# happyjin/Gaussian_process

Measured on AMD Instinct MI355X. Metric: GP-fit+predict sec and achieved fp64 TFLOP/s, N=65536 d=8, 1/2/4/8 MI355X, higher is better.
Workload: dtype f64

## Files before the change

gaussian_process_amd/csrc/gemm_dma.hip:

```cpp
#include <algorithm>
#include <cstdlib>
#include <type_traits>

#include "gpmi_internal.h"
#include "gpmi_plan.h"
#include <atomic>
#include <mutex>

namespace gpmi {

typedef double d4 __attribute__((ext_vector_type(4)));
typedef double d2 __attribute__((ext_vector_type(2)));

#define GPMI_LDS __attribute__((address_space(3)))
#define GPMI_GLB __attribute__((address_space(1)))
#define GPMI_CONST __attribute__((address_space(4)))

struct GemmDmaDev {
    double* C;
    const double* A;
    const double* B;
    int64_t ldc, lda, ldb;
    int Tm, Tn;
    int nchunks;
    int lower;
    int64_t diag_off;
    const int32_t* row_ncols;
    int row_block_tiles;
    const int64_t* b_block_off;
    int b_block_tiles;
    int S, logS, SM, SN, tri, nsuper;
    int pair;
    int sprefix[DMA_MAX_SM + 1];
    unsigned long long* stamps;
    int dbg;
    struct PersistSlot* slot;
    int nblocks;
};

struct PersistSlot {
    unsigned ctr[8];
    unsigned done;
    unsigned pad[7];
};

template <class PT>
__device__ __forceinline__ bool dma_block_to_tile(const PT& p, int b, int& ti, int& tj) {
    return plan_block_to_tile(p, b, ti, tj);
}

__device__ __forceinline__ bool dma_map_tile(const GemmDmaDev& p, int& ti, int& tj) {
    return dma_block_to_tile(p, blockIdx.x, ti, tj);
}

constexpr int DMA_TM = PLAN_TILE, DMA_TN = PLAN_TILE;
template <class PT>
__device__ __forceinline__ bool dma_tile_live(const PT& p, int ti, int tj) {
    return plan_tile_live(p, ti, tj, p.row_ncols);
}
constexpr int DMA_STAGE_SLOTS = (DMA_TM + DMA_TN) * 8;
constexpr int DMA_STAGES = 3;

constexpr unsigned TICKET_NONE = 0xFFFFFFFFu;

template <class PT>
__device__ __forceinline__ unsigned ticket_draw(const PT& p, int xcd) {
    const unsigned per = (unsigned)p.nblocks >> 3;
#pragma unroll 1
    for (int t = 0; t < 8; ++t) {
        const int x = (xcd + t) & 7;
        if (t && __hip_atomic_load(&p.slot->ctr[x], __ATOMIC_RELAXED, __HIP_MEMORY_SCOPE_AGENT) >= per) continue;
        const unsigned w = atomicAdd(&p.slot->ctr[x], 1u);
        if (w < per) return w * 8u + (unsigned)x;
    }
    return TICKET_NONE;
}

template <int MI, bool DBG, bool TICKET = false>
__device__ __forceinline__ void gemm_nt_dma_body(const GemmDmaDev& p) {
    constexpr int NWAVES = 16 / MI;
    constexpr int DPW = 32 / NWAVES;
    constexpr int RPW = DMA_TM / NWAVES;
    constexpr int NFR = MI + 4;
    const int dbg = DBG ? p.dbg : 0;
    extern __shared__ __attribute__((aligned(16))) char smem_raw[];
    const int tid = threadIdx.x;
    volatile GPMI_LDS int* mbox = (volatile GPMI_LDS int*)(smem_raw + DMA_STAGES * DMA_STAGE_SLOTS * 16);
    unsigned blk = blockIdx.x, nxt_blk = TICKET_NONE;
    int par = 0;
    if constexpr (TICKET) {
        if (tid == 0) mbox[0] = (int)ticket_draw(p, (int)(blockIdx.x & 7));
        __syncthreads();
        blk = (unsigned)__builtin_amdgcn_readfirstlane(mbox[0]);
        par = 1;
    }
  for (;;) {
    int ti = 0, tj = 0;
    bool live;
    if constexpr (TICKET) {
        if (blk == TICKET_NONE) break;
        live = dma_block_to_tile(p, (int)blk, ti, tj) && dma_tile_live(p, ti, tj);
        live = __builtin_amdgcn_readfirstlane(live ? 1 : 0) != 0;
        ti = __builtin_amdgcn_readfirstlane(ti);
        tj = __builtin_amdgcn_readfirstlane(tj);
    } else {
        live = dma_map_tile(p, ti, tj) && dma_tile_live(p, ti, tj);
        if (!live) return;
    }
   if (live) {
    unsigned long long st0 = 0, st1 = 0, st2 = 0, st3 = 0;
    if (DBG && (dbg & 16)) st0 = clock64();
    const int lane = tid & 63;
    const int wave = __builtin_amdgcn_readfirstlane(tid >> 6);
    const int wr = (wave >> 1) * (16 * MI);
    const int wc = (wave & 1) * 64;
    const int fr = lane & 15;
    const int fg = lane >> 4;

    const int drow = lane >> 3;
    const int dkp = (lane & 7) ^ (drow & 7);
    const double* a_src = p.A + ((int64_t)ti * DMA_TM + RPW * wave + drow) * p.lda + dkp * 2;
    int64_t b_row0 = (int64_t)tj * DMA_TN * p.ldb;
    if (p.b_block_off) {
        const int blk = tj / p.b_block_tiles;
        b_row0 = p.b_block_off[blk] + (int64_t)(tj - blk * p.b_block_tiles) * DMA_TN * p.ldb;
    }
    const double* b_src = p.B + b_row0 + (int64_t)(RPW * wave + drow) * p.ldb + dkp * 2;
    const int64_t a_step = 8 * p.lda, b_step = 8 * p.ldb;
    GPMI_LDS char* lds = (GPMI_LDS char*)smem_raw;
    const int a_dst = (RPW * wave) * 128;
    const int b_dst = DMA_TM * 128 + (RPW * wave) * 128;

    auto issue_dma_one = [&](int chunk, int q) {
        const int st = chunk % DMA_STAGES;
        GPMI_LDS char* base = lds + st * (DMA_STAGE_SLOTS * 16);
        const int k0 = chunk * 16;
        if (q < DPW / 2)
            __builtin_amdgcn_global_load_lds((const GPMI_GLB void*)(a_src + q * a_step + k0),
                                             (GPMI_LDS void*)(base + a_dst + q * 1024), 16, 0, 0);
        else
            __builtin_amdgcn_global_load_lds((const GPMI_GLB void*)(b_src + (q - DPW / 2) * b_step + k0),
                                             (GPMI_LDS void*)(base + b_dst + (q - DPW / 2) * 1024), 16, 0, 0);
    };
    auto issue_dma = [&](int chunk) {
#pragma unroll
        for (int q = 0; q < DPW; ++q) issue_dma_one(chunk, q);
    };

    const int x7 = fr & 7;
    const int sl0 = fr * 8 + (fg ^ x7);
    const int sl1 = fr * 8 + ((4 + fg) ^ x7);
    const d2* smem = reinterpret_cast<const d2*>(smem_raw);
    auto read_one = [&](int chunk, int half, int q, d2 (&fa)[MI], d2 (&fb)[4]) {
        const d2* sa = smem + (chunk % DMA_STAGES) * DMA_STAGE_SLOTS;
        const d2* sb = sa + DMA_TM * 8;
        const int sl = half ? sl1 : sl0;
        if (q < MI) fa[q] = sa[(wr + 16 * q) * 8 + sl];
        else fb[q - MI] = sb[(wc + 16 * (q - MI)) * 8 + sl];
    };
    auto read_frags = [&](int chunk, int half, d2 (&fa)[MI], d2 (&fb)[4]) {
#pragma unroll
        for (int q = 0; q < NFR; ++q) read_one(chunk, half, q, fa, fb);
    };

    d4 acc[MI][4];
#pragma unroll
    for (int i = 0; i < MI; ++i)
#pragma unroll
        for (int j = 0; j < 4; ++j) acc[i][j] = d4{0., 0., 0., 0.};
    const int nch = p.nchunks;
    d2 fa0[MI], fb0[4], fa1[MI], fb1[4];
    issue_dma(0);
    if (nch > 1) {
        issue_dma(1);
        if constexpr (DPW == 8) asm volatile("s_waitcnt vmcnt(8)" ::: "memory");
        else asm volatile("s_waitcnt vmcnt(4)" ::: "memory");
    } else {
        asm volatile("s_waitcnt vmcnt(0)" ::: "memory");
    }
    __builtin_amdgcn_s_barrier();
    read_frags(0, 0, fa0, fb0);
    if (DBG && (dbg & 16)) st1 = clock64();

#define GPMI_MFMA_X(FA, FB, T) acc[(T) >> 2][(T) & 3] = __builtin_amdgcn_mfma_f64_16x16x4f64(FA[(T) >> 2].x, FB[(T) & 3].x, acc[(T) >> 2][(T) & 3], 0, 0, 0)
#define GPMI_MFMA_Y(FA, FB, T) acc[(T) >> 2][(T) & 3] = __builtin_amdgcn_mfma_f64_16x16x4f64(FA[(T) >> 2].y, FB[(T) & 3].y, acc[(T) >> 2][(T) & 3], 0, 0, 0)
#define GPMI_FENCE() __builtin_amdgcn_sched_barrier(0)
    constexpr int NT = 4 * MI;
    constexpr int NSLOT = NT / 2;

// ... 62 lines not shown
    }
    constexpr int NB3 = MI < 3 ? MI : 3;
    double cv[NB3][4][4];
#pragma unroll
    for (int i = 0; i < NB3; ++i)
#pragma unroll
        for (int j = 0; j < 4; ++j)
#pragma unroll
            for (int v = 0; v < 4; ++v) cv[i][j][v] = *c_ptr(i, j, v);
    if (DBG && (dbg & 16)) {
        asm volatile("s_waitcnt vmcnt(0)" ::: "memory");
        st3 = clock64();
    }
#pragma unroll
    for (int i = 0; i < MI; ++i) {
#pragma unroll
        for (int j = 0; j < 4; ++j)
#pragma unroll
            for (int v = 0; v < 4; ++v) *c_ptr(i, j, v) = cv[i % NB3][j][v] - acc[i][j][v];
        if (i == 0 && MI > 3) {
#pragma unroll
            for (int j = 0; j < 4; ++j)
#pragma unroll
                for (int v = 0; v < 4; ++v) cv[0][j][v] = *c_ptr(3, j, v);
        }
    }
    if (DBG && (dbg & 16)) {
        asm volatile("s_waitcnt vmcnt(0)" ::: "memory");
        const unsigned long long st4 = clock64();
        if (lane == 0 && blockIdx.x < 4096) {
            unsigned long long* o = p.stamps + ((size_t)blockIdx.x * 4 + (wave & 3)) * 4;
            o[0] = st1 - st0; o[1] = st2 - st1; o[2] = st3 - st2; o[3] = st4 - st3;
        }
    }
   }
    if constexpr (!TICKET) {
        return;
    } else {
        if (tid == 0) {
            if (!live) nxt_blk = ticket_draw(p, (int)(blockIdx.x & 7));
            mbox[par] = (int)nxt_blk;
        }
        __syncthreads();
        blk = (unsigned)__builtin_amdgcn_readfirstlane(mbox[par]);
        par ^= 1;
    }
  }
    if constexpr (TICKET) {
        if (tid == 0) {
            __threadfence();
            const unsigned old = atomicAdd(&p.slot->done, 1u);
            if (old == gridDim.x - 1) {
#pragma unroll
                for (int x = 0; x < 8; ++x) p.slot->ctr[x] = 0;
                p.slot->done = 0;
                __threadfence();
            }
        }
    }
}

template <int MI, bool DBG>
__global__ __launch_bounds__(1024 / MI, (MI == 4) ? 2 : 3) void gemm_nt_dma_kernel(const GemmDmaDev p) {
    gemm_nt_dma_body<MI, DBG>(p);
}

__global__ __launch_bounds__(512, 3) void chol_trailing_update_dma_kernel(const GemmDmaDev p) {
    gemm_nt_dma_body<2, false>(p);
}

constexpr int TALL_TM = 2 * DMA_TM;
constexpr int TALL_STAGE_SLOTS = (TALL_TM + DMA_TN) * 8;
constexpr int TALL_STAGES = 2;
constexpr size_t TALL_LDS = (size_t)TALL_STAGES * TALL_STAGE_SLOTS * 16;
static_assert(TALL_LDS == (size_t)DMA_STAGES * DMA_STAGE_SLOTS * 16, "the tall form keeps the LDS footprint");

template <bool DBG>
__device__ __forceinline__ void gemm_nt_dma_tall_body(const GemmDmaDev& p) {
    constexpr int DPW = 6;
    const int dbg = DBG ? p.dbg : 0;
    extern __shared__ __attribute__((aligned(16))) char smem_raw[];
    const int tid = threadIdx.x;
    int ti = 0, tj = 0;
    if (!dma_block_to_tile(p, blockIdx.x, ti, tj)) return;
    bool l0, l1;
    plan_pair_live(p, ti, tj, p.row_ncols, l0, l1);
    ti = __builtin_amdgcn_readfirstlane(ti);
    tj = __builtin_amdgcn_readfirstlane(tj);
    const bool live0 = __builtin_amdgcn_readfirstlane(l0 ? 1 : 0) != 0;
    const bool live1 = __builtin_amdgcn_readfirstlane(l1 ? 1 : 0) != 0;
    if (!live0 && !live1) return;
    unsigned long long st0 = 0, st1 = 0, st2 = 0, st3 = 0;
    if (DBG && (dbg & 16)) st0 = clock64();
    const int lane = tid & 63;
    const int wave = __builtin_amdgcn_readfirstlane(tid >> 6);
    const bool mine = (wave >> 2) ? live1 : live0;
    const int wr = (wave >> 1) * 64;
    const int wc = (wave & 1) * 64;
    const int fr = lane & 15;
    const int fg = lane >> 4;

    const int drow = lane >> 3;
    const int dkp = (lane & 7) ^ (drow & 7);
    const int arow = 32 * wave - ((ti + 1 >= p.Tm && wave >= 4) ? DMA_TM : 0);
    const double* a_row = p.A + ((int64_t)ti * DMA_TM + arow) * p.lda;
    int64_t b_row0 = (int64_t)tj * DMA_TN * p.ldb;
    if (p.b_block_off) {
        const int blk = tj / p.b_block_tiles;
        b_row0 = p.b_block_off[blk] + (int64_t)(tj - blk * p.b_block_tiles) * DMA_TN * p.ldb;
    }
    const double* b_row = p.B + b_row0 + (int64_t)(16 * wave) * p.ldb;
    const unsigned a_lane = (unsigned)((drow * p.lda + dkp * 2) * 8);
    const unsigned b_lane = (unsigned)((drow * p.ldb + dkp * 2) * 8);
    const int64_t a_step = 8 * p.lda, b_step = 8 * p.ldb;
    GPMI_LDS char* lds = (GPMI_LDS char*)smem_raw;
    const int a_dst = (32 * wave) * 128;
    const int b_dst = TALL_TM * 128 + (16 * wave) * 128;
    auto issue_dma_one = [&](int chunk, int q) {
        GPMI_LDS char* base = lds + (chunk & 1) * (TALL_STAGE_SLOTS * 16);
        const int k0 = chunk * 16;
        unsigned off = q < 4 ? a_lane : b_lane;
        asm volatile("" : "+v"(off));
        if (q < 4)
            __builtin_amdgcn_global_load_lds((const GPMI_GLB void*)((const char*)(a_row + q * a_step + k0) + off),
                                             (GPMI_LDS void*)(base + a_dst + q * 1024), 16, 0, 0);
        else
            __builtin_amdgcn_global_load_lds((const GPMI_GLB void*)((const char*)(b_row + (q - 4) * b_step + k0) + off),
                                             (GPMI_LDS void*)(base + b_dst + (q - 4) * 1024), 16, 0, 0);
    };

    const int x7 = fr & 7;
    const int sl0 = fr * 8 + (fg ^ x7);
    const int sl1 = fr * 8 + ((4 + fg) ^ x7);
    const d2* smem = reinterpret_cast<const d2*>(smem_raw);
    auto read_a = [&](int chunk, int half, int i) -> d2 {
        return smem[(chunk & 1) * TALL_STAGE_SLOTS + (wr + 16 * i) * 8 + (half ? sl1 : sl0)];
    };
    auto read_b = [&](int chunk, int half, int j) -> d2 {
        return smem[(chunk & 1) * TALL_STAGE_SLOTS + TALL_TM * 8 + (wc + 16 * j) * 8 + (half ? sl1 : sl0)];
    };

    d4 acc[4][4];
#pragma unroll
    for (int i = 0; i < 4; ++i)
#pragma unroll
        for (int j = 0; j < 4; ++j) acc[i][j] = d4{0., 0., 0., 0.};
    const int nch = p.nchunks;

#define GPMI_MFMA_X(FA, FB, T) acc[(T) >> 2][(T) & 3] = __builtin_amdgcn_mfma_f64_16x16x4f64(FA[(T) >> 2].x, FB[(T) & 3].x, acc[(T) >> 2][(T) & 3], 0, 0, 0)
#define GPMI_MFMA_Y(FA, FB, T) acc[(T) >> 2][(T) & 3] = __builtin_amdgcn_mfma_f64_16x16x4f64(FA[(T) >> 2].y, FB[(T) & 3].y, acc[(T) >> 2][(T) & 3], 0, 0, 0)
#define GPMI_FENCE() __builtin_amdgcn_sched_barrier(0)
    auto kloop = [&](auto live_tag) {
        constexpr bool LIVE = decltype(live_tag)::value;
        d2 fa[4], fb0[4], fb1[4];
#pragma unroll
        for (int q = 0; q < DPW; ++q) issue_dma_one(0, q);
        if (nch > 1) {
#pragma unroll
            for (int q = 0; q < DPW; ++q) issue_dma_one(1, q);
            asm volatile("s_waitcnt vmcnt(6)" ::: "memory");
        } else {
            asm volatile("s_waitcnt vmcnt(0)" ::: "memory");
        }
        __builtin_amdgcn_s_barrier();
        if constexpr (LIVE) {
#pragma unroll
            for (int i = 0; i < 4; ++i) fa[i] = read_a(0, 0, i);
// ... 478 lines not shown
#pragma unroll
        for (int j = 0; j < 2; ++j)
#pragma unroll
            for (int v = 0; v < 4; ++v) *c_ptr(i, j, v) = cv[i][j][v] - acc[i][j][v];
}

bool gemm_small_eligible(const GemmArgs& a) {
    return a.mode == 0 && a.M % SM_T == 0 && a.N % SM_T == 0 && a.K % 16 == 0 && a.K >= 16 && !a.row_ncols && !a.b_block_off;
}

hipError_t launch_gemm_nt_small(hipStream_t s, const GemmArgs& a) {
    GemmSmallDev p;
    p.C = a.C; p.A = a.A; p.B = a.B; p.ldc = a.ldc; p.lda = a.lda; p.ldb = a.ldb;
    p.Tm = (int)(a.M / SM_T); p.Tn = (int)(a.N / SM_T); p.nchunks = (int)(a.K / 16);
    p.lower = a.lower; p.diag_off = a.diag_off;
    constexpr size_t lds8 = (size_t)8 * SM_STAGE_SLOTS * 16, lds3 = (size_t)3 * SM_STAGE_SLOTS * 16;
    static PerDeviceOnce once;
    const hipError_t ea = once.run([&]() -> hipError_t {
        return hipFuncSetAttribute((const void*)gemm_nt_small_kernel<8>, hipFuncAttributeMaxDynamicSharedMemorySize, (int)lds8);
    });
    if (ea != hipSuccess) return ea;
    if (t_small_shallow) hipLaunchKernelGGL(gemm_nt_small_kernel<3>, dim3((unsigned)(p.Tm * p.Tn)), dim3(256), lds3, s, p);
    else hipLaunchKernelGGL(gemm_nt_small_kernel<8>, dim3((unsigned)(p.Tm * p.Tn)), dim3(256), lds8, s, p);
    return hipGetLastError();
}

struct PersistPool {
    static constexpr int SLOTS = 16384;
    PersistSlot* base = nullptr;
    int groups = 0;
    std::atomic<unsigned> head{0};
    PersistSlot* next() { return base + (head.fetch_add(1, std::memory_order_relaxed) % SLOTS); }
};

static PersistPool* persist_pool() {
    static std::mutex mu;
    static PersistPool pools[16];
    int dev = 0;
    if (hipGetDevice(&dev) != hipSuccess || dev < 0 || dev >= 16) return nullptr;
    PersistPool& pl = pools[dev];
    std::lock_guard<std::mutex> lock(mu);
    if (!pl.base) {
        hipDeviceProp_t prop;
        if (hipGetDeviceProperties(&prop, dev) != hipSuccess) return nullptr;
        void* q = nullptr;
        if (hipMalloc(&q, sizeof(PersistSlot) * PersistPool::SLOTS) != hipSuccess) return nullptr;
        if (hipMemset(q, 0, sizeof(PersistSlot) * PersistPool::SLOTS) != hipSuccess) { (void)hipFree(q); return nullptr; }
        pl.groups = (prop.multiProcessorCount / 8) * 8;
        if (pl.groups < 8) { (void)hipFree(q); return nullptr; }
        const void* fns[] = {(const void*)gemm_nt_dma_persist_kernel, (const void*)chol_trailing_update_persist_kernel,
                             (const void*)gemm_nt_dma_ticket_kernel, (const void*)chol_trailing_update_ticket_kernel};
        for (const void* f : fns)
            if (hipFuncSetAttribute(f, hipFuncAttributeMaxDynamicSharedMemorySize,
                                    (int)(DMA_STAGES * DMA_STAGE_SLOTS * 16 + 16)) != hipSuccess) { (void)hipFree(q); return nullptr; }
        pl.base = static_cast<PersistSlot*>(q);
    }
    return &pl;
}

bool gemm_dma_eligible(const GemmArgs& a) {
    return a.mode == 0 && a.N % 128 == 0 && a.M % 128 == 0 && a.K % 16 == 0 && a.K >= 32;
}

hipError_t launch_gemm_nt_dma(hipStream_t s, const GemmArgs& a) {
    GemmDmaDev p;
    p.C = a.C; p.A = a.A; p.B = a.B;
    p.ldc = a.ldc; p.lda = a.lda; p.ldb = a.ldb;
    p.Tm = (int)(a.M / 128); p.Tn = (int)(a.N / 128);
    p.nchunks = (int)(a.K / 16);
    p.lower = a.lower; p.diag_off = a.diag_off;
    p.row_ncols = a.row_ncols; p.row_block_tiles = a.row_block_tiles > 0 ? a.row_block_tiles : 1;
    p.b_block_off = a.b_block_off;
    p.b_block_tiles = a.b_block_off ? (int)(a.b_block_rows / 128) : 1;
    if (a.b_block_off && (a.b_block_rows <= 0 || a.b_block_rows % 128)) return hipErrorInvalidValue;
    const Tuning& tn = tuning();
    TilePlan plan;
    if (!plan_tiles(plan, p.Tm, p.Tn, a.lower, a.diag_off, a.row_ncols != nullptr, a.row_ncols_host, a.row_bands,
                    p.row_block_tiles, 0, false))
        return hipErrorInvalidValue;
    if (plan.nsuper == 0) return hipSuccess;
    const bool eight = tn.gemm_dma_waves == 8 && !(tn.gemm_dbg & 0xff);
    const bool want_ticket = eight && (tn.gemm_ticket >= 2 || (tn.gemm_ticket == 1 && a.role == 1 && gemm_two_streams_active()));
    const bool want_persist = eight && tn.gemm_persist && a.K >= 256 && !gemm_two_streams_active();
    PersistPool* pool = (want_ticket || want_persist) ? persist_pool() : nullptr;
    const bool ticket = want_ticket && pool && plan.nblocks >= pool->groups;
    const bool persist = !ticket && want_persist && pool && plan.nblocks >= 2 * pool->groups;
    if (!ticket && !persist &&
        !plan_tiles(plan, p.Tm, p.Tn, a.lower, a.diag_off, a.row_ncols != nullptr, a.row_ncols_host, a.row_bands,
                    p.row_block_tiles, 0, tn.gemm_balance != 0))
        return hipErrorInvalidValue;
    p.S = plan.S; p.logS = plan.logS; p.SM = plan.SM; p.SN = plan.SN; p.tri = plan.tri; p.nsuper = plan.nsuper;
    p.pair = 0;
    if (plan.tri == 2) std::copy(plan.sprefix, plan.sprefix + plan.SM + 1, p.sprefix);
    const int nblocks = plan.nblocks;
    constexpr size_t lds = (size_t)DMA_STAGES * DMA_STAGE_SLOTS * 16;
    static PerDeviceOnce once;
    const hipError_t ea = once.run([&]() -> hipError_t {
        const void* fns[] = {(const void*)gemm_nt_dma_kernel<4, false>, (const void*)gemm_nt_dma_kernel<4, true>,
                             (const void*)gemm_nt_dma_kernel<2, false>, (const void*)gemm_nt_dma_kernel<2, true>,
                             (const void*)chol_trailing_update_dma_kernel};
        for (const void* f : fns) {
            const hipError_t e = hipFuncSetAttribute(f, hipFuncAttributeMaxDynamicSharedMemorySize, (int)lds);
            if (e != hipSuccess) return e;
        }
        return hipSuccess;
    });
    if (ea != hipSuccess) return ea;
    p.dbg = tn.gemm_dbg & 0xff;
    p.stamps = tn.gemm_stamps;
    p.slot = nullptr;
    p.nblocks = nblocks;
    if (ticket) {
        p.slot = pool->next();
        constexpr size_t ldst = lds + 16;
        if (a.role == 1) hipLaunchKernelGGL(chol_trailing_update_ticket_kernel, dim3(pool->groups), dim3(512), ldst, s, p);
        else hipLaunchKernelGGL(gemm_nt_dma_ticket_kernel, dim3(pool->groups), dim3(512), ldst, s, p);
        return hipGetLastError();
    }
    if (persist) {
        p.slot = pool->next();
        constexpr size_t ldsp = lds + 16;
        if (a.role == 1) hipLaunchKernelGGL(chol_trailing_update_persist_kernel, dim3(pool->groups), dim3(512), ldsp, s, p);
        else hipLaunchKernelGGL(gemm_nt_dma_persist_kernel, dim3(pool->groups), dim3(512), ldsp, s, p);
        return hipGetLastError();
    }
    if (tn.gemm_dma_waves == 8 && tn.gemm_tall &&
        plan_live_tiles(p.Tm, p.Tn, a.lower, a.diag_off, a.row_ncols_host, a.row_bands, p.row_block_tiles) >= tn.tall_min_tiles) {
        TilePlan pp;
        if (!plan_tiles(pp, p.Tm, p.Tn, a.lower, a.diag_off, a.row_ncols != nullptr, a.row_ncols_host, a.row_bands,
                        p.row_block_tiles, 0, tn.gemm_balance != 0, true))
            return hipErrorInvalidValue;
        p.S = pp.S; p.logS = pp.logS; p.SM = pp.SM; p.SN = pp.SN; p.tri = pp.tri; p.nsuper = pp.nsuper; p.pair = 1;
        if (pp.tri == 2) std::copy(pp.sprefix, pp.sprefix + pp.SM + 1, p.sprefix);
        p.nblocks = pp.nblocks;
        static PerDeviceOnce once_tall;
        const hipError_t et = once_tall.run([&]() -> hipError_t {
            const void* fns[] = {(const void*)gemm_nt_dma_tall_kernel<false>, (const void*)gemm_nt_dma_tall_kernel<true>,
                                 (const void*)chol_trailing_update_dma256_kernel};
            for (const void* f : fns) {
                const hipError_t e = hipFuncSetAttribute(f, hipFuncAttributeMaxDynamicSharedMemorySize, (int)TALL_LDS);
                if (e != hipSuccess) return e;
            }
            return hipSuccess;
        });
        if (et != hipSuccess) return et;
        if (p.dbg) hipLaunchKernelGGL(gemm_nt_dma_tall_kernel<true>, dim3(pp.nblocks), dim3(512), TALL_LDS, s, p);
        else if (a.role == 1) hipLaunchKernelGGL(chol_trailing_update_dma256_kernel, dim3(pp.nblocks), dim3(512), TALL_LDS, s, p);
        else hipLaunchKernelGGL(gemm_nt_dma_tall_kernel<false>, dim3(pp.nblocks), dim3(512), TALL_LDS, s, p);
        return hipGetLastError();
    }
    if (tn.gemm_dma_waves == 8) {
        if (p.dbg) hipLaunchKernelGGL((gemm_nt_dma_kernel<2, true>), dim3(nblocks), dim3(512), lds, s, p);
        else if (a.role == 1) hipLaunchKernelGGL(chol_trailing_update_dma_kernel, dim3(nblocks), dim3(512), lds, s, p);
        else hipLaunchKernelGGL((gemm_nt_dma_kernel<2, false>), dim3(nblocks), dim3(512), lds, s, p);
    } else {
        if (p.dbg) hipLaunchKernelGGL((gemm_nt_dma_kernel<4, true>), dim3(nblocks), dim3(256), lds, s, p);
        else hipLaunchKernelGGL((gemm_nt_dma_kernel<4, false>), dim3(nblocks), dim3(256), lds, s, p);
    }
    return hipGetLastError();
}

}
```

gaussian_process_amd/csrc/gpmi_api.hip:

```cpp
#include "gpmi_ctx.h"

using namespace gpmi;

namespace gpmi {
thread_local std::string g_err;

static thread_local Tuning t_dev_tuning;
static thread_local const Tuning* t_tuning = nullptr;
const Tuning& tuning() { return t_tuning ? *t_tuning : t_dev_tuning; }
TuneScope::TuneScope(const Tuning* t) : prev(t_tuning) { t_tuning = t; }
TuneScope::~TuneScope() { t_tuning = prev; }
}

extern "C" {

int gpmi_abi_version(void) { return GPMI_ABI_VERSION; }
const char* gpmi_last_error(void) { return g_err.c_str(); }

int gpmi_device_count(int* count) {
    if (!count) return fail_arg("gpmi_device_count: null pointer");
    int n = 0;
    hipError_t e = hipGetDeviceCount(&n);
    if (e != hipSuccess) { *count = 0; return fail_runtime(e, "hipGetDeviceCount"); }
    *count = n;
    return GPMI_OK;
}

int gpmi_ctx_create(int device, gpmi_ctx** out) {
    if (!out) return fail_arg("gpmi_ctx_create: null out pointer");
    *out = nullptr;
    int n = 0;
    HIP_TRY(hipGetDeviceCount(&n));
    if (device < 0 || device >= n) return fail_arg("gpmi_ctx_create: no such device");
    HIP_TRY(hipSetDevice(device));
    gpmi_ctx* c = new gpmi_ctx();
    c->device = device;
    int prio_lo = 0, prio_hi = 0;
    (void)hipDeviceGetStreamPriorityRange(&prio_lo, &prio_hi);
    hipError_t e = hipStreamCreateWithPriority(&c->stream, hipStreamNonBlocking, prio_lo);
    if (e != hipSuccess) { delete c; return fail_runtime(e, "hipStreamCreate"); }
    e = hipStreamCreateWithPriority(&c->pstream, hipStreamNonBlocking, prio_hi);
    if (e != hipSuccess) { (void)hipStreamDestroy(c->stream); delete c; return fail_runtime(e, "hipStreamCreate"); }
    const char* env;
    if ((env = getenv("GPMI_NB"))) c->nb = std::max<int64_t>(128, atoll(env) / 128 * 128);
    if ((env = getenv("GPMI_LD_PAD"))) c->ld_pad = std::max<int64_t>(0, atoll(env) / 2 * 2);
    if ((env = getenv("GPMI_LOOKAHEAD"))) c->lookahead = atoi(env) ? 1 : 0;
    *out = c;
    return GPMI_OK;
}

int gpmi_ctx_destroy(gpmi_ctx* c) {
    if (!c) return GPMI_OK;
    for (gpmi_ctx* l : c->lane_ctx) (void)gpmi_ctx_destroy(l);
    c->lane_ctx.clear();
    (void)hipSetDevice(c->device);
    (void)hipStreamSynchronize(c->stream);
    for (DevBuf* b : {&c->X, &c->y, &c->A, &c->info, &c->red, &c->Xs, &c->V, &c->P, &c->vec, &c->dense,
                       &c->U, &c->Kn, &c->gpart, &c->cov_a, &c->cov_b, &c->cov_out, &c->flag, &c->vside,
                       &c->lap, &c->lap_part, &c->lap_out})
        b->release();
    for (auto e : c->ev_pool) (void)hipEventDestroy(e);
    (void)hipStreamDestroy(c->stream);
    (void)hipStreamDestroy(c->pstream);
    if (c->vstream) (void)hipStreamDestroy(c->vstream);
    delete c;
    return GPMI_OK;
}

static int set_tuning_option(Tuning& t, const char* name, int64_t value) {
    if (!strcmp(name, "gemm_small_tiles")) {
        t.gemm_small_tiles = value ? 1 : 0;
    } else if (!strcmp(name, "trsm_wave")) {
        t.trsm_wave = value ? 1 : 0;
    } else if (!strcmp(name, "gemm_small_dma")) {
        t.gemm_small_dma = value ? 1 : 0;
    } else if (!strcmp(name, "gemm_persist")) {
        t.gemm_persist = value ? 1 : 0;
    } else if (!strcmp(name, "gemm_ticket")) {
        if (value < 0 || value > 2) return fail_arg("gemm_ticket must be 0 (off), 1 (trailing updates under lookahead) or 2 (every launch)");
        t.gemm_ticket = (int)value;
    } else if (!strcmp(name, "gemm_balance")) {
        t.gemm_balance = value ? 1 : 0;
    } else if (!strcmp(name, "trsv_vinv")) {
        if (value < 0 || value > 2) return fail_arg("trsv_vinv must be 0 (16 x 16 rounds), 1 (one launch per block) or 2 (one launch)");
        t.trsv_vinv = (int)value;
    } else if (!strcmp(name, "panel_fused")) {
        t.panel_fused = value ? 1 : 0;
    } else if (!strcmp(name, "rbf_blocks")) {
        if (value < 1 || value > (1 << 24)) return fail_arg("rbf_blocks must be in 1..2^24");
        t.rbf_blocks = (int)value;
    } else if (!strcmp(name, "gemm_dma_waves")) {
        if (value != 4 && value != 8) return fail_arg("gemm_dma_waves must be 4 or 8");
        t.gemm_dma_waves = (int)value;
    } else if (!strcmp(name, "gemm_tall")) {
        if (value < 0 || value > 1) return fail_arg("gemm_tall must be 0 (128 x 128 blocks) or 1 (256 x 128 blocks for large launches)");
        t.gemm_tall = (int)value;
    } else if (!strcmp(name, "tall_min_tiles")) {
        if (value < 0 || value > (1 << 30)) return fail_arg("tall_min_tiles must be in 0..2^30");
        t.tall_min_tiles = (int)value;
    } else if (!strcmp(name, "gemm_dma")) {
        t.gemm_use_dma = value ? 1 : 0;
    } else {
        return -1;
    }
    return GPMI_OK;
}

int gpmi_set_option(gpmi_ctx* c, const char* name, int64_t value) {
    if (!c || !name) return fail_arg("gpmi_set_option: null argument");
    if (!strcmp(name, "nb")) {
        if (value != 0 && (value < 128 || value % 128)) return fail_arg("nb must be 0 (auto) or a positive multiple of 128");
        c->nb = value;
    } else if (!strcmp(name, "ld_pad")) {
        if (value < 0 || value % 2) return fail_arg("ld_pad must be even and >= 0");
        c->ld_pad = value;
        c->have_factor = c->have_v = c->have_laplace = false;
    } else if (!strcmp(name, "timing")) {
        c->timing = value ? 1 : 0;
    } else if (!strcmp(name, "lookahead")) {
        c->lookahead = value ? 1 : 0;
    } else if (!strcmp(name, "la_min")) {
        if (value < 0) return fail_arg("la_min must be >= 0");
        c->la_min = value;
    } else if (!strcmp(name, "shallow_min")) {
        if (value < 0) return fail_arg("shallow_min must be >= 0");
        c->shallow_min = value;
    } else if (!strcmp(name, "one_pass_form")) {
        if (value < 0 || value > 2) return fail_arg("one_pass_form must be 0 (by size), 1 (rows ride) or 2 (rows follow)");
        c->one_pass_form = (int)value;
    } else if (!strcmp(name, "lanes")) {
        if (value < 0 || value > 8) return fail_arg("lanes must be 0 (by size) .. 8");
        c->lanes = (int)value;
    } else if (!strcmp(name, "ramp")) {
        if (value < 0 || (value & 8) || (value >> 4) > 64) return fail_arg("ramp: bits 0-2 and a tail count of at most 64 in bits 4..");
        c->ramp = (int)value;
    } else {
        const int rc = set_tuning_option(c->tune, name, value);
        if (rc < 0) return fail_arg("gpmi_set_option: unknown option");
        return rc;
    }
    return GPMI_OK;
}

int gpmi_dev_set_option(const char* name, int64_t value) {
    if (!name) return fail_arg("gpmi_dev_set_option: null argument");
    const int rc = set_tuning_option(t_dev_tuning, name, value);
    if (rc < 0) return fail_arg("gpmi_dev_set_option: unknown option");
    return rc;
}

int gpmi_set_kernel(gpmi_ctx* c, int kind, double p0, double p1) {
    if (!c) return fail_arg("gpmi_set_kernel: null context");
    if (kind < 0 || kind > 2) return fail_arg("gpmi_set_kernel: kind must be 0 (rbf), 1 (linear) or 2 (periodic)");
    if (kind == 2 && (!(p0 != 0.0) || !(p1 != 0.0))) return fail_arg("gpmi_set_kernel: period and lengthscale must be non-zero");
    c->kind = kind; c->kp0 = p0; c->kp1 = p1;
    c->have_factor = c->have_v = c->have_laplace = false;
    return GPMI_OK;
}

int gpmi_set_kernel_params(gpmi_ctx* c, int kind, const double* params, int nparams) {
    if (!c || !params) return fail_arg("gpmi_set_kernel_params: null argument");
    if (kind != 3) {
        if (kind < 0 || kind > 2 || nparams != 2) return fail_arg("gpmi_set_kernel_params: kinds 0-2 take 2 parameters");
// ... 634 lines not shown
```

gaussian_process_amd/csrc/gpmi_internal.h:

```cpp
#pragma once
#include <hip/hip_runtime.h>
#include <stdint.h>

#include <mutex>

namespace gpmi {

constexpr int TILE = 128;
constexpr int IB = 64;

struct Tuning {
    int gemm_use_dma = 1;
    int gemm_small_tiles = 1;
    int gemm_persist = 1;
    int gemm_ticket = 0;
    int gemm_balance = 1;
    int gemm_dma_waves = 8;
    int gemm_tall = 1;
    int tall_min_tiles = 12288;
    int trsm_wave = 1;
    int rbf_blocks = 16384;
    int trsv_vinv = 2;
    int panel_fused = 1;
    int gemm_small_dma = 1;
    int gemm_dbg = 0;
    unsigned long long* gemm_stamps = nullptr;
    unsigned long long* panel_stamps = nullptr;
};
const Tuning& tuning();
struct TuneScope {
    const Tuning* prev;
    explicit TuneScope(const Tuning* t);
    ~TuneScope();
};

struct PerDeviceOnce {
    std::mutex mu;
    uint64_t done = 0;
    template <class F> hipError_t run(F fn) {
        int dev = 0;
        hipError_t e = hipGetDevice(&dev);
        if (e != hipSuccess) return e;
        std::lock_guard<std::mutex> lock(mu);
        if (dev < 64 && ((done >> dev) & 1)) return hipSuccess;
        e = fn();
        if (e == hipSuccess && dev < 64) done |= (uint64_t)1 << dev;
        return e;
    }
};

struct GemmArgs {
    double* C;
    const double* A;
    const double* B;
    int64_t ldc, lda, ldb;
    int64_t M, N, K;
    int mode;
    int lower;
    int64_t diag_off;
    const int32_t* row_ncols = nullptr;
    int row_block_tiles = 1;
    const int32_t* row_ncols_host = nullptr;
    int row_bands = 0;
    int role = 0;
    const int64_t* b_block_off = nullptr;
    int64_t b_block_rows = 0;
};
hipError_t launch_gemm_nt(hipStream_t s, const GemmArgs& a);
bool gemm_nt_routes_dma(const GemmArgs& a);
double gemm_nt_algorithmic_flops(const GemmArgs& a, int64_t real_rows);
bool gemm_dma_eligible(const GemmArgs& a);
hipError_t launch_gemm_nt_dma(hipStream_t s, const GemmArgs& a);
bool gemm_small_eligible(const GemmArgs& a);
bool gemm_shallow_active();
bool gemm_two_streams_active();
struct GemmShallowScope {
    int prev, prev_two;
    explicit GemmShallowScope(bool on, bool two_streams = false, bool exact = false);
    ~GemmShallowScope();
};
hipError_t launch_gemm_nt_small(hipStream_t s, const GemmArgs& a);
double gemm_nt_flops(const GemmArgs& a);

hipError_t launch_potf2_64(hipStream_t s, double* A, int64_t ld, int64_t col_offset,
                           int64_t* info_dev);
hipError_t launch_trsm_rlt64(hipStream_t s, const double* L, int64_t ldl, double* X, int64_t ldx,
                             int64_t m);

hipError_t launch_potrf128(hipStream_t s, double* A, int64_t ld, int64_t col_offset, int64_t* info_dev);

hipError_t launch_trsm128(hipStream_t s, const double* L, int64_t ldl, double* X, int64_t ldx, int64_t m);

struct RbfArgs {
    const double* A;
    const double* B;
    int64_t nA, nB, d;
    int64_t row0;
    int64_t nrows;
// ... 66 lines not shown
```

gaussian_process_amd/csrc/gpmi_plan.h:

```cpp
#pragma once
#include <math.h>
#include <stdint.h>

#include <algorithm>
#include <vector>

#if defined(__HIPCC__)
#define GPMI_HD __host__ __device__ __forceinline__
#else
#define GPMI_HD inline
#endif

namespace gpmi {

constexpr int PLAN_TILE = 128;
constexpr int DMA_MAX_SM = 128;

struct TilePlan {
    int Tm = 0, Tn = 0;
    int lower = 0;
    int64_t diag_off = 0;
    int row_block_tiles = 1;
    int S = 1, logS = 0, SM = 0, SN = 0;
    int tri = 0;
    int nsuper = 0;
    int nblocks = 0;
    int pair = 0;
    int sprefix[DMA_MAX_SM + 1];
    const int32_t* row_ncols = nullptr;
};

template <class PT>
GPMI_HD bool plan_block_to_tile(const PT& p, int b, int& ti, int& tj) {
    const int xcd = b & 7;
    const int w = b >> 3;
    const int S2 = (p.S * p.S) >> p.pair;
    const int s = (w / S2) * 8 + xcd;
    if (s >= p.nsuper) return false;
    const int q = w % S2;
    int si, sj;
    if (p.tri == 2) {
        si = 0;
        while (si + 1 < p.SM && p.sprefix[si + 1] <= s) ++si;
        sj = s - p.sprefix[si];
        if (sj == p.sprefix[si + 1] - p.sprefix[si] - 1 && p.row_ncols) {
            int acc = 0;
            for (int r = 0; r < (p.S >> p.pair); ++r) {
                const int tr = si * p.S + (r << p.pair);
                int w = 0;
                for (int h = 0; h <= p.pair; ++h) {
                    if (tr + h >= p.Tm) break;
                    const int64_t nc = p.row_ncols[(tr + h) / p.row_block_tiles];
                    int64_t wl = (nc + PLAN_TILE - 1) / PLAN_TILE - (int64_t)sj * p.S;
                    if (wl > p.S) wl = p.S;
                    if (wl > (int64_t)p.Tn - (int64_t)sj * p.S) wl = (int64_t)p.Tn - (int64_t)sj * p.S;
                    if (wl > w) w = (int)wl;
                }
                if (q < acc + w) {
                    ti = tr;
                    tj = sj * p.S + (q - acc);
                    return true;
                }
                acc += w;
            }
            return false;
        }
    } else if (p.tri) {
        si = (int)((sqrtf(8.f * (float)s + 1.f) - 1.f) * 0.5f);
        while ((si + 1) * (si + 2) / 2 <= s) ++si;
        while (si * (si + 1) / 2 > s) --si;
        sj = s - si * (si + 1) / 2;
    } else {
        si = s / p.SN;
        sj = s - si * p.SN;
        sj += si % p.SN;
        if (sj >= p.SN) sj -= p.SN;
    }
    if (p.tri == 1 && si == sj && p.pair) {
        int r = (int)((sqrtf(4.f * (float)q + 1.f) - 1.f) * 0.5f);
        while ((r + 1) * (r + 2) <= q) ++r;
        while (r * (r + 1) > q) --r;
        if (2 * r >= p.S) return false;
        ti = si * p.S + 2 * r;
        tj = sj * p.S + (q - r * (r + 1));
        return ti < p.Tm && tj < p.Tn;
    }
    if (p.tri == 1 && si == sj) {
        int r = (int)((sqrtf(8.f * (float)q + 1.f) - 1.f) * 0.5f);
        while ((r + 1) * (r + 2) / 2 <= q) ++r;
        while (r * (r + 1) / 2 > q) --r;
        if (r >= p.S) return false;
        ti = si * p.S + r;
        tj = sj * p.S + (q - r * (r + 1) / 2);
// ... 30 lines not shown
inline double plan_xcd_efficiency(const TilePlan& p, const int32_t* row_ncols_host, int cus_per_engine = 8) {
    long load[32];
    for (int x = 0; x < 32; ++x) load[x] = 0;
    long total = 0;
    for (int b = 0; b < p.nblocks; ++b) {
        int ti, tj;
        if (!plan_block_to_tile(p, b, ti, tj)) continue;
        bool l0, l1 = false;
        if (p.pair) plan_pair_live(p, ti, tj, row_ncols_host, l0, l1);
        else l0 = plan_tile_live(p, ti, tj, row_ncols_host);
        if (l0 || l1) { ++load[b & 31]; total += (long)l0 + (long)l1; }
    }
    long rounds = 0;
    for (int x = 0; x < 32; ++x) rounds = std::max(rounds, (load[x] + cus_per_engine - 1) / cus_per_engine);
    return rounds ? (double)total / (32.0 * cus_per_engine * (1 + p.pair)) / (double)rounds : 1.0;
}

inline bool plan_tiles(TilePlan& p, int64_t Tm, int64_t Tn, int lower, int64_t diag_off, bool has_row_map,
                       const int32_t* row_ncols_host, int row_bands, int row_block_tiles, int force_S,
                       bool balance_xcds, bool pair) {
    if (Tm <= 0 || Tn <= 0 || Tm > (1 << 20) || Tn > (1 << 20)) return false;
    if (row_ncols_host && row_bands <= 0) return false;
    p.Tm = (int)Tm; p.Tn = (int)Tn;
    p.lower = lower; p.diag_off = diag_off;
    p.row_block_tiles = row_block_tiles > 0 ? row_block_tiles : 1;
    p.tri = (lower && diag_off == 0 && 2 * p.Tn >= p.Tm) ? 1 : 0;
    p.row_ncols = nullptr;
    p.pair = pair ? 1 : 0;
    const bool stairs = has_row_map && row_ncols_host && row_bands > 0 && !lower;
    int S = 8;
    while (S > 1 && (S > p.Tn || S > p.Tm)) S >>= 1;
    const int min_S = pair ? 2 : 1;
    if (S < min_S) S = min_S;
    if (force_S && force_S < min_S) return false;
    if (!force_S && balance_xcds && S > 2 &&
        ((p.tri == 1 && !stairs && p.Tn <= 256) || (stairs && (int64_t)p.Tm * p.Tn <= 32768))) {
        double eff[4] = {0., 0., 0., 0.}, best = 0.0;
        int cand[4], nc = 0;
        for (int c = S; c >= 2 && nc < 4; c >>= 1) {
            TilePlan q;
            if (!plan_tiles(q, Tm, Tn, lower, diag_off, has_row_map, row_ncols_host, row_bands, row_block_tiles, c, false, pair)) break;
            if (stairs && q.tri != 2) break;
            cand[nc] = c;
            eff[nc] = plan_xcd_efficiency(q, row_ncols_host);
            best = std::max(best, eff[nc]);
            ++nc;
        }
        for (int i = 0; i < nc; ++i)
            if (eff[i] >= best - 0.01) { force_S = cand[i]; break; }
    }
    if (force_S) S = force_S;
    for (;; S >>= 1) {
        const int SM = (p.Tm + S - 1) / S, SN = (p.Tn + S - 1) / S;
        int ns = p.tri ? SM * (SM + 1) / 2 : SM * SN;
        bool use_stairs = false;
        if (stairs && SM <= DMA_MAX_SM) {
            int tot = 0;
            p.sprefix[0] = 0;
            for (int si = 0; si < SM; ++si) {
                int64_t widest = 0;
                for (int ti = si * S; ti < std::min((si + 1) * S, p.Tm); ++ti) {
                    const int band = std::min(ti / p.row_block_tiles, row_bands - 1);
                    widest = std::max<int64_t>(widest, row_ncols_host[band]);
                }
                widest = std::max<int64_t>(widest, 0);
                const int64_t live = std::min<int64_t>(SN, (widest + (int64_t)S * PLAN_TILE - 1) / ((int64_t)S * PLAN_TILE));
                tot += (int)live;
                p.sprefix[si + 1] = tot;
            }
            ns = tot;
            use_stairs = true;
        }
        if (ns >= 32 || S == min_S || force_S) {
            p.S = S; p.SM = SM; p.SN = SN; p.nsuper = ns;
            if (use_stairs) { p.tri = 2; p.row_ncols = row_ncols_host; }
            break;
        }
    }
    p.logS = (p.S == 8) ? 3 : (p.S == 4) ? 2 : (p.S == 2) ? 1 : 0;
    p.nblocks = ((p.nsuper + 7) / 8) * 8 * ((p.S * p.S) >> p.pair);
    return true;
}

inline int64_t plan_live_tiles(int64_t Tm, int64_t Tn, int lower, int64_t diag_off, const int32_t* row_ncols_host,
                               int row_bands, int row_block_tiles) {
    int64_t n = 0;
    const int rbt = row_block_tiles > 0 ? row_block_tiles : 1;
    for (int64_t ti = 0; ti < Tm; ++ti) {
        int64_t w = Tn;
        if (lower) {
            const int64_t lim = ti * PLAN_TILE + PLAN_TILE - 1 + diag_off;
            w = lim < 0 ? 0 : std::min<int64_t>(Tn, lim / PLAN_TILE + 1);
        }
        if (row_ncols_host && row_bands > 0) {
            const int64_t nc = row_ncols_host[std::min<int64_t>(ti / rbt, row_bands - 1)];
            w = std::min<int64_t>(w, nc > 0 ? (nc + PLAN_TILE - 1) / PLAN_TILE : 0);
        }
        n += w;
    }
    return n;
}

inline std::vector<int64_t> plan_block_widths(int64_t NB, int64_t ncols, bool ramp_ok, int ramp) {
    std::vector<int64_t> w;
    if (NB <= 0 || ncols <= 0) return w;
    const bool on = ramp_ok && ramp && NB >= 1024 && ncols >= 8 * NB;
    const bool up = on && (ramp & 1), down = on && (ramp & 2);
    const int64_t tail = (ramp >> 4) ? (ramp >> 4) : 3;
    int64_t done = 0;
    while (done < ncols) {
        int64_t nb = NB;
        const int64_t left = ncols - done;
        if (up && w.size() < 2) nb = NB / 4;
        else if (up && w.size() < 3) nb = NB / 2;
        else if (down && left <= NB && (ramp & 4)) nb = NB / 4;
        else if (down && left <= tail * NB) nb = NB / 2;
        nb = std::min(nb, ncols - done);
        w.push_back(nb);
        done += nb;
    }
    return w;
}

inline double plan_tile_flops(int64_t M, int64_t N, int64_t K, int lower, int64_t diag_off) {
    if (M <= 0 || N <= 0 || K <= 0) return 0.;
    const int TN = (N % 128 == 0) ? 128 : 64;
    const int64_t Tm = M / 128, Tn = N / TN;
    int64_t tiles = 0;
    for (int64_t ti = 0; ti < Tm; ++ti) {
        if (!lower) { tiles += Tn; continue; }
        const int64_t lim = ti * 128 + 127 + diag_off;
        if (lim < 0) continue;
        const int64_t cnt = lim / TN + 1;
        tiles += cnt < Tn ? cnt : Tn;
    }
    return 2.0 * (double)tiles * 128.0 * TN * (double)K;
}

inline double plan_algorithmic_flops(int64_t M, int64_t N, int64_t K, int lower, int64_t diag_off, int64_t real_rows) {
    if (M <= 0 || N <= 0 || K <= 0) return 0.;
    const int64_t rows = std::min<int64_t>(M, real_rows);
    if (!lower) return 2.0 * (double)rows * (double)N * (double)K;
    double elems = 0.;
    const int64_t r_full = std::max<int64_t>(0, N - 1 - diag_off);
    const int64_t r_first = std::max<int64_t>(0, -diag_off);
    const int64_t tri_end = std::min(rows, r_full);
    if (tri_end > r_first) {
        const double n = (double)(tri_end - r_first);
        const double first = (double)(r_first + diag_off + 1);
        elems += n * first + n * (n - 1) / 2.0;
    }
    if (rows > r_full) elems += (double)(rows - std::max(r_full, (int64_t)0)) * (double)N;
    return 2.0 * elems * (double)K;
}

}
```

Before: 68.36.

## Assign GEMM tiles by per-XCD atomic draw with slack grid for trailing updates

Adds a dynamic tile-draw mode in which each block of the non-persistent DMA GEMM kernels takes its tile index from per-XCD atomic counters instead of using blockIdx. The grid gets a small slack of extra blocks, and the last block resets the counters. It is on by default for trailing Cholesky updates under two-stream lookahead, and it disables static balancing in that mode. The aim is to absorb uneven tile progress when these launches share the GPU with another stream. The cost is extra atomics, two block-wide barriers per block, and idle slack blocks.

```diff
diff --git a/gaussian_process_amd/csrc/gemm_dma.hip b/gaussian_process_amd/csrc/gemm_dma.hip
--- a/gaussian_process_amd/csrc/gemm_dma.hip
+++ b/gaussian_process_amd/csrc/gemm_dma.hip
@@ -49,10 +49,6 @@
     return plan_block_to_tile(p, b, ti, tj);
 }
 
-__device__ __forceinline__ bool dma_map_tile(const GemmDmaDev& p, int& ti, int& tj) {
-    return dma_block_to_tile(p, blockIdx.x, ti, tj);
-}
-
 constexpr int DMA_TM = PLAN_TILE, DMA_TN = PLAN_TILE;
 template <class PT>
 __device__ __forceinline__ bool dma_tile_live(const PT& p, int ti, int tj) {
@@ -61,19 +57,47 @@
 constexpr int DMA_STAGE_SLOTS = (DMA_TM + DMA_TN) * 8;
 constexpr int DMA_STAGES = 3;
 
-constexpr unsigned TICKET_NONE = 0xFFFFFFFFu;
+constexpr unsigned TICKET_NONE = PLAN_DRAW_NONE;
 
 template <class PT>
 __device__ __forceinline__ unsigned ticket_draw(const PT& p, int xcd) {
-    const unsigned per = (unsigned)p.nblocks >> 3;
-#pragma unroll 1
-    for (int t = 0; t < 8; ++t) {
-        const int x = (xcd + t) & 7;
-        if (t && __hip_atomic_load(&p.slot->ctr[x], __ATOMIC_RELAXED, __HIP_MEMORY_SCOPE_AGENT) >= per) continue;
-        const unsigned w = atomicAdd(&p.slot->ctr[x], 1u);
-        if (w < per) return w * 8u + (unsigned)x;
-    }
-    return TICKET_NONE;
+    unsigned* ctr = p.slot->ctr;
+    return plan_draw((unsigned)p.nblocks, xcd,
+                     [&](int x) { return __hip_atomic_load(&ctr[x], __ATOMIC_RELAXED, __HIP_MEMORY_SCOPE_AGENT); },
+                     [&](int x) { return atomicAdd(&ctr[x], 1u); });
+}
+
+template <class PT>
+__device__ __forceinline__ unsigned drawn_block(const PT& p) {
+    extern __shared__ __attribute__((aligned(16))) char smem_raw[];
+    volatile GPMI_LDS unsigned* mbox = (volatile GPMI_LDS unsigned*)smem_raw;
+    if (threadIdx.x == 0) {
+        unsigned* ctr = p.slot->ctr;
+        unsigned snap[8];
+        bool have = false;
+        const unsigned b = plan_draw((unsigned)p.nblocks, (int)(blockIdx.x & 7),
+                                     [&](int x) {
+                                         if (!have) {
+#pragma unroll
+                                             for (int i = 0; i < 8; ++i)
+                                                 snap[i] = __hip_atomic_load(&ctr[i], __ATOMIC_RELAXED, __HIP_MEMORY_SCOPE_AGENT);
+                                             have = true;
+                                         }
+                                         return snap[x];
+                                     },
+                                     [&](int x) { return atomicAdd(&ctr[x], 1u); });
+        mbox[0] = b;
+        __atomic_signal_fence(__ATOMIC_SEQ_CST);
+        if (atomicAdd(&p.slot->done, 1u) == gridDim.x - 1) {
+#pragma unroll
+            for (int x = 0; x < 8; ++x) __hip_atomic_store(&p.slot->ctr[x], 0u, __ATOMIC_RELAXED, __HIP_MEMORY_SCOPE_AGENT);
+            __hip_atomic_store(&p.slot->done, 0u, __ATOMIC_RELAXED, __HIP_MEMORY_SCOPE_AGENT);
+        }
+    }
+    __syncthreads();
+    const unsigned b = (unsigned)__builtin_amdgcn_readfirstlane((int)mbox[0]);
+    __syncthreads();
+    return b;
 }
 
 template <int MI, bool DBG, bool TICKET = false>
@@ -104,7 +128,11 @@
         ti = __builtin_amdgcn_readfirstlane(ti);
         tj = __builtin_amdgcn_readfirstlane(tj);
     } else {
-        live = dma_map_tile(p, ti, tj) && dma_tile_live(p, ti, tj);
+        if (p.slot) {
+            blk = drawn_block(p);
+            if (blk == TICKET_NONE) return;
+        }
+        live = dma_block_to_tile(p, (int)blk, ti, tj) && dma_tile_live(p, ti, tj);
         if (!live) return;
     }
    if (live) {
@@ -333,7 +361,12 @@
     extern __shared__ __attribute__((aligned(16))) char smem_raw[];
     const int tid = threadIdx.x;
     int ti = 0, tj = 0;
-    if (!dma_block_to_tile(p, blockIdx.x, ti, tj)) return;
+    unsigned blk = blockIdx.x;
+    if (p.slot) {
+        blk = drawn_block(p);
+        if (blk == TICKET_NONE) return;
+    }
+    if (!dma_block_to_tile(p, (int)blk, ti, tj)) return;
     bool l0, l1;
     plan_pair_live(p, ti, tj, p.row_ncols, l0, l1);
     ti = __builtin_amdgcn_readfirstlane(ti);
@@ -978,12 +1011,15 @@
     const bool eight = tn.gemm_dma_waves == 8 && !(tn.gemm_dbg & 0xff);
     const bool want_ticket = eight && (tn.gemm_ticket >= 2 || (tn.gemm_ticket == 1 && a.role == 1 && gemm_two_streams_active()));
     const bool want_persist = eight && tn.gemm_persist && a.K >= 256 && !gemm_two_streams_active();
-    PersistPool* pool = (want_ticket || want_persist) ? persist_pool() : nullptr;
+    const bool want_draw = eight && (tn.gemm_draw >= 2 || (tn.gemm_draw == 1 && a.role == 1 && gemm_two_streams_active()));
+    PersistPool* pool = (want_ticket || want_persist || want_draw) ? persist_pool() : nullptr;
     const bool ticket = want_ticket && pool && plan.nblocks >= pool->groups;
     const bool persist = !ticket && want_persist && pool && plan.nblocks >= 2 * pool->groups;
+    const bool draw = !ticket && !persist && want_draw && pool;
+    const bool balance = tn.gemm_balance != 0 && !draw;
     if (!ticket && !persist &&
         !plan_tiles(plan, p.Tm, p.Tn, a.lower, a.diag_off, a.row_ncols != nullptr, a.row_ncols_host, a.row_bands,
-                    p.row_block_tiles, 0, tn.gemm_balance != 0))
+                    p.row_block_tiles, 0, balance))
         return hipErrorInvalidValue;
     p.S = plan.S; p.logS = plan.logS; p.SM = plan.SM; p.SN = plan.SN; p.tri = plan.tri; p.nsuper = plan.nsuper;
     p.pair = 0;
@@ -1024,7 +1060,7 @@
         plan_live_tiles(p.Tm, p.Tn, a.lower, a.diag_off, a.row_ncols_host, a.row_bands, p.row_block_tiles) >= tn.tall_min_tiles) {
         TilePlan pp;
         if (!plan_tiles(pp, p.Tm, p.Tn, a.lower, a.diag_off, a.row_ncols != nullptr, a.row_ncols_host, a.row_bands,
-                        p.row_block_tiles, 0, tn.gemm_balance != 0, true))
+                        p.row_block_tiles, 0, balance, true))
             return hipErrorInvalidValue;
         p.S = pp.S; p.logS = pp.logS; p.SM = pp.SM; p.SN = pp.SN; p.tri = pp.tri; p.nsuper = pp.nsuper; p.pair = 1;
         if (pp.tri == 2) std::copy(pp.sprefix, pp.sprefix + pp.SM + 1, p.sprefix);
@@ -1040,15 +1076,19 @@
             return hipSuccess;
         });
         if (et != hipSuccess) return et;
-        if (p.dbg) hipLaunchKernelGGL(gemm_nt_dma_tall_kernel<true>, dim3(pp.nblocks), dim3(512), TALL_LDS, s, p);
-        else if (a.role == 1) hipLaunchKernelGGL(chol_trailing_update_dma256_kernel, dim3(pp.nblocks), dim3(512), TALL_LDS, s, p);
-        else hipLaunchKernelGGL(gemm_nt_dma_tall_kernel<false>, dim3(pp.nblocks), dim3(512), TALL_LDS, s, p);
+        const unsigned grid = (unsigned)(draw ? plan_draw_grid(pp.nblocks, tn.gemm_draw_slack) : pp.nblocks);
+        if (draw) p.slot = pool->next();
+        if (p.dbg) hipLaunchKernelGGL(gemm_nt_dma_tall_kernel<true>, dim3(grid), dim3(512), TALL_LDS, s, p);
+        else if (a.role == 1) hipLaunchKernelGGL(chol_trailing_update_dma256_kernel, dim3(grid), dim3(512), TALL_LDS, s, p);
+        else hipLaunchKernelGGL(gemm_nt_dma_tall_kernel<false>, dim3(grid), dim3(512), TALL_LDS, s, p);
         return hipGetLastError();
     }
     if (tn.gemm_dma_waves == 8) {
-        if (p.dbg) hipLaunchKernelGGL((gemm_nt_dma_kernel<2, true>), dim3(nblocks), dim3(512), lds, s, p);
-        else if (a.role == 1) hipLaunchKernelGGL(chol_trailing_update_dma_kernel, dim3(nblocks), dim3(512), lds, s, p);
-        else hipLaunchKernelGGL((gemm_nt_dma_kernel<2, false>), dim3(nblocks), dim3(512), lds, s, p);
+        const unsigned grid = (unsigned)(draw ? plan_draw_grid(nblocks, tn.gemm_draw_slack) : nblocks);
+        if (draw) p.slot = pool->next();
+        if (p.dbg) hipLaunchKernelGGL((gemm_nt_dma_kernel<2, true>), dim3(grid), dim3(512), lds, s, p);
+        else if (a.role == 1) hipLaunchKernelGGL(chol_trailing_update_dma_kernel, dim3(grid), dim3(512), lds, s, p);
+        else hipLaunchKernelGGL((gemm_nt_dma_kernel<2, false>), dim3(grid), dim3(512), lds, s, p);
     } else {
         if (p.dbg) hipLaunchKernelGGL((gemm_nt_dma_kernel<4, true>), dim3(nblocks), dim3(256), lds, s, p);
         else hipLaunchKernelGGL((gemm_nt_dma_kernel<4, false>), dim3(nblocks), dim3(256), lds, s, p);
diff --git a/gaussian_process_amd/csrc/gpmi_api.hip b/gaussian_process_amd/csrc/gpmi_api.hip
--- a/gaussian_process_amd/csrc/gpmi_api.hip
+++ b/gaussian_process_amd/csrc/gpmi_api.hip
@@ -79,6 +79,12 @@
     } else if (!strcmp(name, "gemm_ticket")) {
         if (value < 0 || value > 2) return fail_arg("gemm_ticket must be 0 (off), 1 (trailing updates under lookahead) or 2 (every launch)");
         t.gemm_ticket = (int)value;
+    } else if (!strcmp(name, "gemm_draw")) {
+        if (value < 0 || value > 2) return fail_arg("gemm_draw must be 0 (off), 1 (trailing updates under lookahead) or 2 (every per-tile launch)");
+        t.gemm_draw = (int)value;
+    } else if (!strcmp(name, "gemm_draw_slack")) {
+        if (value < 0 || value > 400) return fail_arg("gemm_draw_slack must be in 0..400 (percent)");
+        t.gemm_draw_slack = (int)value;
     } else if (!strcmp(name, "gemm_balance")) {
         t.gemm_balance = value ? 1 : 0;
     } else if (!strcmp(name, "trsv_vinv")) {
diff --git a/gaussian_process_amd/csrc/gpmi_internal.h b/gaussian_process_amd/csrc/gpmi_internal.h
--- a/gaussian_process_amd/csrc/gpmi_internal.h
+++ b/gaussian_process_amd/csrc/gpmi_internal.h
@@ -14,6 +14,8 @@
     int gemm_small_tiles = 1;
     int gemm_persist = 1;
     int gemm_ticket = 0;
+    int gemm_draw = 1;
+    int gemm_draw_slack = 8;
     int gemm_balance = 1;
     int gemm_dma_waves = 8;
     int gemm_tall = 1;
diff --git a/gaussian_process_amd/csrc/gpmi_plan.h b/gaussian_process_amd/csrc/gpmi_plan.h
--- a/gaussian_process_amd/csrc/gpmi_plan.h
+++ b/gaussian_process_amd/csrc/gpmi_plan.h
@@ -7,8 +7,10 @@
 
 #if defined(__HIPCC__)
 #define GPMI_HD __host__ __device__ __forceinline__
+#define GPMI_NO_UNROLL _Pragma("unroll 1")
 #else
 #define GPMI_HD inline
+#define GPMI_NO_UNROLL
 #endif
 
 namespace gpmi {
@@ -205,6 +207,26 @@
     return true;
 }
 
+constexpr unsigned PLAN_DRAW_NONE = 0xFFFFFFFFu;
+
+inline int64_t plan_draw_grid(int64_t nblocks, int slack_pct) {
+    const int64_t per = nblocks / 8;
+    return 8 * ((per * (100 + (int64_t)slack_pct) + 99) / 100);
+}
+
+template <class Load, class Add>
+GPMI_HD unsigned plan_draw(unsigned nblocks, int xcd, Load load, Add add) {
+    const unsigned per = nblocks >> 3;
+    GPMI_NO_UNROLL
+    for (int t = 0; t < 8; ++t) {
+        const int x = (xcd + t) & 7;
+        if (t && load(x) >= per) continue;
+        const unsigned w = add(x);
+        if (w < per) return w * 8u + (unsigned)x;
+    }
+    return PLAN_DRAW_NONE;
+}
+
 inline int64_t plan_live_tiles(int64_t Tm, int64_t Tn, int lower, int64_t diag_off, const int32_t* row_ncols_host,
                                int row_bands, int row_block_tiles) {
     int64_t n = 0;
```

Measured after the change: 69.30 (median of 6 runs). +1.4%, better.
